# nordmtr/quantpy

Measured on AMD Instinct MI355X. Metric: state reconstructions/sec (3-qubit MLE), higher is better.
Workload: dtype f64

## Files before the change

quantpy_amd/csrc/qt_small.h:

```cpp
#pragma once
#include <hip/hip_runtime.h>
#include <stdint.h>

#include <type_traits>

#include "qt_linesearch.h"

namespace qt {

#ifdef QT_PHASE_TIMING
__device__ long long* g_qt_prof = nullptr;
#define QT_PROF_ROW \
  ((size_t)(blockIdx.x + threadIdx.y * gridDim.x) * (blockDim.x >> 6) + (threadIdx.x >> 6))
#define QT_STAMP(slot)                                                                                   \
  do {                                                                                                   \
    if (g_qt_prof && (threadIdx.x & 63) == 0)                                                            \
      g_qt_prof[QT_PROF_ROW * 32 + (slot)] = (long long)__builtin_readcyclecounter();                    \
  } while (0)
#define QT_STAMP_VAL(slot, val)                                                                          \
  do {                                                                                                   \
    if (g_qt_prof && (threadIdx.x & 63) == 0)                                                            \
      g_qt_prof[QT_PROF_ROW * 32 + (slot)] = (val);                                                      \
  } while (0)
#else
// ... 220 lines not shown
struct EstOut {
  double* rho;
  const double* centre;
  double* dist;
};

template <int NQ>
struct Small {
  static constexpr int d = 1 << NQ;
  static constexpr int D = d * d;
  static constexpr int G = D;
  static constexpr int TPW = 64 / G;
  static constexpr int WPB = 4;
  static constexpr int NT = 64 * WPB;
  static constexpr int TPB = TPW * WPB;
  static constexpr int T = d * (d - 1) / 2;
  static constexpr int LD = d == 8 ? 9 : d;
  static constexpr int MAT = 2 * LD * d;
  static constexpr int oA = 0;
  static constexpr int oB = oA + MAT;
  static constexpr int oVec = oB + MAT;
  static constexpr int oLam = oVec + D + 2;
  static constexpr int oM = oLam + 2 * ((d + 1) / 2);
  __host__ __device__ static bool v_on_rbuf(int M) { return ((M + 1) & ~1) >= MAT; }
  __host__ __device__ static int v_offset(int M, int R1) {
    const int Mp = (M + 1) & ~1;
    return v_on_rbuf(M) ? oM : oM + (R1 > 0 ? 3 : 2) * Mp;
  }
  __host__ __device__ static int trial_doubles(int M, int R1 = 0) {
    const int Mp = (M + 1) & ~1;
    return oM + (R1 > 0 ? 3 : 2) * Mp + (v_on_rbuf(M) ? 0 : MAT);
  }
  __host__ __device__ static int ipow_h(int b, int e) {
    int r = 1;
    for (int t = 0; t < e; ++t) r *= b;
    return r;
  }
  __host__ __device__ static int fwd_ints(int R1) {
    int t = 0;
    for (int q = 1; q <= NQ; ++q) t += ipow_h(R1, q) << (2 * (NQ - q));
    return t;
  }
  __host__ __device__ static int bwd_ints(int R1) {
    int t = 0;
    for (int q = 1; q <= NQ; ++q) t += ipow_h(R1, q - 1) << (2 * (NQ - q + 1));
    return t;
  }
  __host__ __device__ static int table_ints(int M, int R1) { return (fwd_ints(R1) + bwd_ints(R1) + M + 1) & ~1; }
  __host__ __device__ static int table_doubles(int M, int R1) {
    return R1 > 0 ? (table_ints(M, R1) / 2 + ((M + 1) & ~1) + 8 * R1) : 0;
  }
  __host__ __device__ static size_t lds_bytes(int M, int R1 = 0, int extra = 0) {
    return ((size_t)table_doubles(M, R1) + (size_t)TPB * (trial_doubles(M, R1) + extra)) * sizeof(double);
  }

  struct Ctx {
    int l, i, j, e;
    double* sm;
    const int *tfwd, *tbwd, *trmap;
    const double* twrow;
    const double *ttab, *ptab;
    int M, Mp;
    PovmView pv;
    int xm, zm, ny;
    int pi, pj, pkind;
    int src_re, src_im;
    __device__ __forceinline__ cd* A() const { return reinterpret_cast<cd*>(sm + oA); }
    __device__ __forceinline__ cd* Bm() const { return reinterpret_cast<cd*>(sm + oB); }
    __device__ __forceinline__ cd* V() const { return reinterpret_cast<cd*>(sm + v_offset(M, pv.pr.enabled ? pv.pr.R1 : 0)); }
    __device__ __forceinline__ double* vec() const { return sm + oVec; }
    __device__ __forceinline__ double* lam() const { return sm + oLam; }
    __device__ __forceinline__ double* rbuf() const { return sm + oM; }
    __device__ __forceinline__ double* freq() const { return sm + oM + Mp; }
    __device__ __forceinline__ double* bufB() const { return sm + oM + 2 * Mp; }
    __device__ __forceinline__ const double* tabT() const { return ttab; }
    __device__ __forceinline__ const double* tabP() const { return ptab; }
    __device__ __forceinline__ bool prod() const { return pv.pr.enabled != 0; }
    __device__ __forceinline__ double* extra() const { return sm + trial_doubles(M, pv.pr.enabled ? pv.pr.R1 : 0); }
    static constexpr bool kGeneric = true;
    static constexpr bool kHelper = false;
    __device__ __forceinline__ static constexpr int verdict_load() { return 0; }
    __device__ __forceinline__ static constexpr bool abandoned(int) { return false; }
    __device__ __forceinline__ int R1() const { return pv.pr.R1; }
    __device__ __forceinline__ bool uniform() const { return pv.pr.uniform != 0; }
    __device__ __forceinline__ bool pairedT() const { return pv.pr.pairedT != 0; }
    __device__ __forceinline__ bool pairedP() const { return pv.pr.pairedP != 0; }
    __device__ __forceinline__ double wuni() const { return pv.pr.wuni; }
    __device__ __forceinline__ double jtol2() const { return pv.jtol2; }
    __device__ __forceinline__ double cT(int k) const { return pv.pr.cT[k]; }
    __device__ __forceinline__ double cP(int k) const { return pv.pr.cP[k]; }
  };
  struct CtxS {
    int l, i, j, e;
    double* sm;
    const int* tfwd;
    const double *ttab, *ptab;
    int M, Mp;
    SpecArgs a;
    int xm, zm, ny;
    int pi, pj, pkind;
    int src_re, src_im;
    int bslot;
    double kT[12], kP[12];
    __device__ __forceinline__ cd* A() const { return reinterpret_cast<cd*>(sm + oA); }
    __device__ __forceinline__ cd* Bm() const { return reinterpret_cast<cd*>(sm + oB); }
    __device__ __forceinline__ cd* V() const { return reinterpret_cast<cd*>(sm + v_offset(M, 6)); }
    __device__ __forceinline__ double* vec() const { return sm + oVec; }
    __device__ __forceinline__ double* lam() const { return sm + oLam; }
    __device__ __forceinline__ double* rbuf() const { return sm + oM; }
    __device__ __forceinline__ double* freq() const { return sm + oM + Mp; }
    __device__ __forceinline__ double* bufB() const { return sm + oM + 2 * Mp; }
    __device__ __forceinline__ const double* tabT() const { return ttab; }
    __device__ __forceinline__ const double* tabP() const { return ptab; }
    __device__ __forceinline__ double* extra() const { return sm + trial_doubles(M, 6); }
    static constexpr bool kGeneric = false;
    static constexpr bool kHelper = false;
    __device__ __forceinline__ static constexpr int verdict_load() { return 0; }
    __device__ __forceinline__ static constexpr bool abandoned(int) { return false; }
    __device__ __forceinline__ static constexpr bool prod() { return true; }
    __device__ __forceinline__ static constexpr int R1() { return 6; }
    __device__ __forceinline__ static constexpr bool uniform() { return true; }
    __device__ __forceinline__ static constexpr bool pairedT() { return true; }
    __device__ __forceinline__ static constexpr bool pairedP() { return true; }
    __device__ __forceinline__ double wuni() const { return a.wuni; }
    __device__ __forceinline__ double jtol2() const { return a.jtol2; }
    __device__ __forceinline__ double cT(int k) const { return kT[k]; }
    __device__ __forceinline__ double cP(int k) const { return kP[k]; }
  };
  __device__ __forceinline__ static double pin_vgpr(double x) {
    asm volatile("" : "+v"(x));
    return x;
  }
  template <bool GENERIC, class = void>
  struct CtxOf {
    using type = Ctx;
  };
  template <class X>
  struct CtxOf<false, X> {
    using type = CtxS;
  };
  __host__ __device__ static int image_last_ints(int M) { return (M + 3) & ~3; }
  __host__ __device__ static int image_chunks(int M) { return image_last_ints(M) / 4 + 2 * 24 / 2; }

  __device__ __forceinline__ static int trial_index(int B, bool* live) {
    const int wave = threadIdx.x >> 6, tib = (threadIdx.x & 63) / G;
    const int b = (blockIdx.x * WPB + wave) * TPW + tib;
    *live = b < B;
    return b;
  }

  __device__ static void make_ctx(Ctx& c, double* smem_block, const PovmView& pv) {
    const int lane = threadIdx.x & 63, wave = threadIdx.x >> 6;
    c.l = lane % G;
    const int slot = wave * TPW + lane / G;
    c.i = c.l / d;
    c.j = c.l % d;
    c.e = c.i * LD + c.j;
    c.M = pv.M;
    c.Mp = (pv.M + 1) & ~1;
    c.pv = pv;
    const int r1 = pv.pr.enabled ? pv.pr.R1 : 0;
    int* tabs = reinterpret_cast<int*>(smem_block);
    c.tfwd = tabs;
    c.tbwd = tabs + fwd_ints(r1);
    c.trmap = c.tbwd + bwd_ints(r1);
    double* wrow = smem_block + table_ints(pv.M, r1) / 2;
    double* t1 = wrow + ((pv.M + 1) & ~1);
    c.twrow = wrow;
    c.ttab = t1;
    c.ptab = t1 + 4 * r1;
    if (r1 > 0) {
      const int nf = fwd_ints(r1), nb = bwd_ints(r1);
      for (int e = threadIdx.x; e < 4 * r1; e += NT) {
        t1[e] = pv.pr.T[e];
        t1[4 * r1 + e] = pv.pr.P1T[e];
      }
      if (pv.pr.pairedT) {
        for (int e = threadIdx.x; e < pv.M; e += NT) tabs[e] = pv.pr.last[e];
      } else {
        for (int e = threadIdx.x; e < nf; e += NT) tabs[e] = pv.pr.fwd[e];
      }
      if (!(pv.pr.pairedT && pv.pr.pairedP))
        for (int e = threadIdx.x; e < nb; e += NT) tabs[nf + e] = pv.pr.bwd[e];
      for (int e = threadIdx.x; e < pv.M; e += NT) {
        tabs[nf + nb + e] = pv.pr.rmap[e];
        wrow[e] = pv.pr.wrowR[e];
      }
      __syncthreads();
    }
    c.sm = smem_block + table_doubles(pv.M, r1) + slot * (trial_doubles(pv.M, r1) + pv.extra);
    int xm = 0, zm = 0, ny = 0;
#pragma unroll
    for (int b = 0; b < NQ; ++b) {
      const int dig = (c.l >> (2 * b)) & 3;
      if (dig == 1 || dig == 2) xm |= 1 << b;
      if (dig == 2 || dig == 3) zm |= 1 << b;
      if (dig == 2) ++ny;
    }
    c.xm = xm;
    c.zm = zm;
    c.ny = ny & 3;
    if (c.l < d) {
      c.pi = c.pj = c.l;
      c.pkind = 0;
    } else {
      int t = c.l - d;
      c.pkind = 1;
      if (t >= T) {
        t -= T;
        c.pkind = 2;
      }
      int ii = 1;
      while ((ii * (ii + 1)) / 2 <= t) ++ii;
      c.pi = ii;
      c.pj = t - (ii * (ii - 1)) / 2;
    }
    c.src_re = c.src_im = D;
    if (c.i == c.j) c.src_re = c.i;
    else if (c.i > c.j) {
      const int tt = (c.i * (c.i - 1)) / 2 + c.j;
      c.src_re = d + tt;
      c.src_im = d + T + tt;
    }
    if (c.l == 0) c.sm[oVec + D] = 0.0;
  }

  __device__ __forceinline__ static int pauli_index(int x, int z) {
    int k = 0;
#pragma unroll
    for (int b = 0; b < NQ; ++b) {
      const int xb = (x >> b) & 1, zb = (z >> b) & 1;
      const int dig = xb ? (zb ? 2 : 1) : (zb ? 3 : 0);
      k |= dig << (2 * b);
    }
    return k;
  }
  __device__ __forceinline__ static double re_phase(int ny, cd s) {
    return ny == 0 ? s.re : ny == 1 ? s.im : ny == 2 ? -s.re : -s.im;
  }
  __device__ __forceinline__ static cd phase_times(int ny, double v) {
    return ny == 0 ? cd{v, 0.0} : ny == 1 ? cd{0.0, -v} : ny == 2 ? cd{-v, 0.0} : cd{0.0, v};
  }

// ... 143 lines not shown
        }
      }
      wave_sync();
#pragma unroll
      for (int q = 0; q < 4; ++q) {
        const int m = c.l + q * G, mc = m < c.M ? m : c.M - 1;
        fq[mc] = raw[c.prod() ? c.trmap[mc] : mc] * inv;
      }
    } else {
      for (int m = c.l; m < c.M; m += G) {
        const double v = (double)counts[m];
        raw[m] = v;
        part += v;
      }
      total = gsum<G>(part);
      inv = 1.0 / total;
      wave_sync();
      if (c.prod()) {
        for (int m = c.l; m < c.M; m += G) fq[m] = raw[c.trmap[m]] * inv;
      } else {
        for (int m = c.l; m < c.M; m += G) fq[m] = raw[m] * inv;
      }
    }
    if (c.pv.Ns && !(pf && pf->seg)) {
      const int K = c.pv.K;
      for (int s = c.l; s < c.pv.S; s += G) {
        double t = 0.0;
        for (int k = 0; k < K; ++k) t += raw[s * K + k];
        const double ns = (pf && s == c.l) ? pf->ns[0] : c.pv.Ns[s];
        bad |= !shots_match(t, total, ns, c.pv.ns_tot);
      }
    }
    const unsigned long long votes = __builtin_amdgcn_ballot_w64(bad);
    const int lane = threadIdx.x & 63;
    const unsigned long long mine = (G == 64) ? ~0ull : (((1ull << (G & 63)) - 1ull) << (lane / G * G));
    wave_sync();
    return (votes & mine) == 0ull;
  }

  __device__ __forceinline__ static void prefetch_counts(Prefetch& pf, const int64_t* counts, const SpecArgs& a) {
    const int l = (threadIdx.x & 63) % G, M = a.M, nch = image_chunks(M), t = threadIdx.x;
    const uint4* img = reinterpret_cast<const uint4*>(a.image);
    const int* rinv = reinterpret_cast<const int*>(img + nch);
    pf.img = img[t < nch ? t : nch - 1];
    pf.ok = pf.seg = true;
#pragma unroll
    for (int q = 0; q < 4; ++q) {
      const int m = l + q * G, mc = m < M ? m : M - 1;
      pf.v[q] = counts[mc];
      pf.ri[q] = rinv[mc];
      pf.ns[q] = a.Ns[mc >> NQ];
    }
  }
  template <bool VCOEF = false>
  __device__ static void make_ctx(CtxS& c, double* smem_block, const SpecArgs& a, const Prefetch& pf) {
    const int lane = threadIdx.x & 63, wave = threadIdx.x >> 6;
    c.l = lane % G;
    const int slot = wave * TPW + lane / G;
    c.i = c.l / d;
    c.j = c.l % d;
    c.e = c.i * LD + c.j;
    c.M = a.M;
    c.Mp = (a.M + 1) & ~1;
    c.a = a;
    if ((int)threadIdx.x < image_chunks(a.M)) reinterpret_cast<uint4*>(smem_block)[threadIdx.x] = pf.img;
    c.tfwd = reinterpret_cast<const int*>(smem_block);
    c.ttab = smem_block + image_last_ints(a.M) / 2;
    c.ptab = c.ttab + 24;
    c.sm = smem_block + table_doubles(a.M, 6) + slot * (trial_doubles(a.M, 6) + a.extra);
    if (c.l == 0) c.sm[oVec + D] = 0.0;
    __syncthreads();
    int xm = 0, zm = 0, ny = 0;
#pragma unroll
    for (int b = 0; b < NQ; ++b) {
      const int dig = (c.l >> (2 * b)) & 3;
      xm |= (dig == 1 || dig == 2) << b;
      zm |= (dig >= 2) << b;
      ny += dig == 2;
    }
    c.xm = xm;
    c.zm = zm;
    c.ny = ny & 3;
    param_owner(c.l, c.pi, c.pj, c.pkind);
    const int tt = (c.i * (c.i - 1)) / 2 + c.j;
    c.src_re = c.i == c.j ? c.i : c.i > c.j ? d + tt : D;
    c.src_im = c.i > c.j ? d + T + tt : D;
    const int sx = (c.i & 1) | ((c.i & 2) << 1) | ((c.i & 4) << 2), sz = (c.j & 1) | ((c.j & 2) << 1) | ((c.j & 4) << 2);
    c.bslot = sx ^ (3 * sz);
#pragma unroll
    for (int k = 0; k < 12; ++k) {
      c.kT[k] = VCOEF ? pin_vgpr(a.cT[k]) : a.cT[k];
      c.kP[k] = VCOEF ? pin_vgpr(a.cP[k]) : a.cP[k];
    }
  }
  template <int KK>
  __device__ __forceinline__ static double gsum_above(double v) {
    if (KK < 2) v += dpp_f64<0xB1>(v);
    if (KK < 4) v += dpp_f64<0x4E>(v);
    if (G >= 8 && KK < 8) v += dpp_f64<0x141>(v);
    if (G >= 16 && KK < 16) v += dpp_f64<0x140>(v);
    if (G == 64) {
      v += dpp_f64<0x142, 0xA>(v);
      v += dpp_f64<0x143, 0xC>(v);
      v = readlane_f64(v, 63);
    }
    return v;
  }
  __device__ static bool load_freq(const CtxS& c, const Prefetch& pf) {
    double dv[4], st[4];
    bool valid[4];
#pragma unroll
    for (int q = 0; q < 4; ++q) {
      valid[q] = c.l + q * G < c.M;
      dv[q] = valid[q] ? (double)pf.v[q] : 0.0;
      st[q] = segsum_c<d>(dv[q]);
    }
    const double total = gsum_above<d>((st[0] + st[1]) + (st[2] + st[3]));
    const double inv = 1.0 / total;
    bool bad = false;
#pragma unroll
    for (int q = 0; q < 4; ++q) bad |= valid[q] & !shots_match(st[q], total, pf.ns[q], c.a.ns_tot);
    double* fq = c.freq();
// ... 327 lines not shown
        const double piv = readlane_f64(b.re, k * d + k);
        const cd bip = Vs[i * LD + k], bpj = Vs[k * LD + j];
        double inv = __builtin_amdgcn_rcp(piv);
        inv = fma(inv, fma(-piv, inv, 1.0), inv);
        inv = fma(inv, fma(-piv, inv, 1.0), inv);
        const cd t{bpj.re * inv, bpj.im * inv};
        const cd e = cmul(bip, t);
        cd nb{b.re - e.re, b.im - e.im};
        if (j == k) nb = cd{-bip.re * inv, -bip.im * inv};
        if (i == k) nb = (j == k) ? cd{inv, 0.0} : t;
        b = nb;
        if (k + 1 < d) Vs[c.e] = b;
      }
      const double mag = fabs(akk);
      const bool pos = akk > 0.0;
      if (!pos) {
        if (neg == 0) kneg = k;
        ++neg;
      }
      if (!(mag > 1e-13)) neg = neg > 0 ? 99 : neg;
      const double safe = mag > 1e-300 ? mag : 1e-300;
      if (k + 1 < d) {
        const double inv = recip_nr(safe);
        const double sinv = pos ? -inv : inv;
        const cd ajs{ajk.re * sinv, ajk.im * sinv};
        const bool upd = i > k && j > k;
        const double nre = fma(aik.re, ajs.re, fma(aik.im, ajs.im, a.re));
        const double nim = fma(aik.im, ajs.re, fma(-aik.re, ajs.im, a.im));
        a.re = upd ? nre : a.re;
        a.im = upd ? nim : a.im;
        A[c.e] = a;
        wave_sync();
      }
    }
    {
      const double dj = A[j * LD + j].re;
      const double mj = fabs(dj);
      const double rs = fast_rsqrt(mj > 1e-300 ? mj : 1e-300);
      if (i >= j) lmine = (i == j) ? cd{dj * rs, 0.0} : cd{a.re * rs, a.im * rs};
    }
    ok = neg == 0;
    if (neg_out) *neg_out = neg;
    if (kneg_out) *kneg_out = kneg;
    if (SPEC && spec_inv) *spec_inv = b;
    L[c.e] = lmine;
    wave_sync();
    const cd e = L[c.pi * LD + c.pj];
    const double x = c.pkind == 2 ? e.im : e.re;
    wave_sync();
    return x;
  }

  struct HelperLink {
    enum : int { kUnset = 0, kSpec = 1 };
    enum : int { kPending = 0, kGo = 1, kAbort = 2, kClaimed = 3, kRevoked = 4 };
    enum : int { kNothing = 0, kLifted = 1, kRefused = 2 };
    static constexpr int kHelperPolls = 1 << 15, kWaitPolls = 1 << 14, kClaimedPolls = 1 << 16;
    double* base;
    int pending;
    __device__ __forceinline__ static constexpr int doubles() { return 2 * MAT + D + 3; }
    __device__ __forceinline__ cd* image(int k) const { return reinterpret_cast<cd*>(base + k * MAT); }
    __device__ __forceinline__ cd* result() const { return image(1); }
    __device__ __forceinline__ double* x() const { return base + 2 * MAT; }
    __device__ __forceinline__ int* task() const { return reinterpret_cast<int*>(base + 2 * MAT + D); }
    __device__ __forceinline__ int* verdict() const { return task() + 1; }
    __device__ __forceinline__ int* lifted() const { return task() + 2; }
    __device__ __forceinline__ int* done() const { return task() + 3; }
    __device__ __forceinline__ int* gone() const { return task() + 4; }
    __device__ __forceinline__ int* ok() const { return task() + 5; }
    __device__ __forceinline__ static void publish(int* w, int v) {
      wave_sync();
      if ((threadIdx.x & 63) == 0) __hip_atomic_store(w, v, __ATOMIC_RELEASE, __HIP_MEMORY_SCOPE_WORKGROUP);
    }
    __device__ __forceinline__ static int peek(const int* w) {
      return __builtin_amdgcn_readfirstlane(__hip_atomic_load(w, __ATOMIC_RELAXED, __HIP_MEMORY_SCOPE_WORKGROUP));
    }
    __device__ __forceinline__ static bool claim(int* w, int from, int to) {
      int won = 0;
      if ((threadIdx.x & 63) == 0) {
        int expect = from;
        won = __hip_atomic_compare_exchange_strong(w, &expect, to, __ATOMIC_ACQ_REL, __ATOMIC_RELAXED,
                                                   __HIP_MEMORY_SCOPE_WORKGROUP);
      }
      return __builtin_amdgcn_readfirstlane(won) != 0;
    }
    template <int SLEEP>
    __device__ __forceinline__ static int poll(const int* w, int idle, int polls) {
      int v = idle;
#pragma unroll 1
      for (int n = 0; n < polls; ++n) {
        v = peek(w);
        if (v != idle) break;
        __builtin_amdgcn_s_sleep(SLEEP);
      }
      return v;
    }
    __device__ __forceinline__ void reset() {
      pending = 0;
      if ((threadIdx.x & 63) == 0) {
        *task() = kUnset;
        *verdict() = kPending;
        *lifted() = kNothing;
        *done() = 0;
        *gone() = 0;
      }
    }
    __device__ __forceinline__ void speculate(int e, cd lin) const {
      image(0)[e] = lin;
      publish(task(), kSpec);
    }
    __device__ __forceinline__ void decide(bool go) const { publish(verdict(), go ? kGo : kAbort); }
    __device__ __forceinline__ int await_lift(int e, cd& proj) {
      int v = poll<1>(lifted(), kNothing, kWaitPolls);
      if (v == kNothing) {
        if (claim(verdict(), kGo, kRevoked)) return kNothing;
        v = poll<1>(lifted(), kNothing, kClaimedPolls);
        if (v == kNothing) return kNothing;
      }
      __builtin_amdgcn_fence(__ATOMIC_ACQUIRE, "workgroup");
      if (v == kLifted) {
        proj = result()[e];
        pending = 1;
      }
      return v;
    }
    __device__ __forceinline__ bool collect(int l, double& xl, int& okl) const {
      if (poll<1>(done(), 0, kClaimedPolls) == 0) return false;
      __builtin_amdgcn_fence(__ATOMIC_ACQUIRE, "workgroup");
      xl = x()[l];
      okl = *ok();
      return true;
    }
    __device__ __forceinline__ void await_gone() const {
      poll<1>(gone(), 0, kClaimedPolls);
      __builtin_amdgcn_fence(__ATOMIC_ACQUIRE, "workgroup");
    }
  };
  struct CtxH {
    int l, i, j, e, pi, pj, pkind;
    cd *image, *second, *factor;
    const int* verdict;
    __device__ __forceinline__ cd* A() const { return image; }
    __device__ __forceinline__ cd* Bm() const { return factor; }
    __device__ __forceinline__ cd* V() const { return second; }
    __device__ __forceinline__ int verdict_load() const {
      return __hip_atomic_load(verdict, __ATOMIC_RELAXED, __HIP_MEMORY_SCOPE_WORKGROUP);
    }
    __device__ __forceinline__ static bool abandoned(int v) {
      v = __builtin_amdgcn_readfirstlane(v);
      return v != HelperLink::kPending && v != HelperLink::kGo;
    }
  };
  struct LateX {
    bool got;
    double x;
    int ok;
  };
  template <class Base>
  struct WithHelper : Base {
    HelperLink* link;
    LateX* late;
    static constexpr bool kHelper = true;
  };
  __device__ __forceinline__ static void param_owner(int l, int& pi, int& pj, int& pkind) {
    const bool diag = l < d, imag = l >= d + T;
    const int t = l - d - (imag ? T : 0);
    int ii = 1;
#pragma unroll
    for (int k = 2; k < d; ++k) ii += t >= (k * (k - 1)) / 2;
    pkind = diag ? 0 : imag ? 2 : 1;
    pi = diag ? l : ii;
    pj = diag ? l : t - (ii * (ii - 1)) / 2;
  }
  __device__ static void helper_wave(const HelperLink& k, cd* L) {
    helper_work(k, L);
    HelperLink::publish(k.gone(), 1);
  }
  __device__ static void helper_work(const HelperLink& k, cd* L) {
    static_assert(G == 64, "one trial per wavefront");
    if (HelperLink::template poll<2>(k.task(), HelperLink::kUnset, HelperLink::kHelperPolls) != HelperLink::kSpec) return;
    __builtin_amdgcn_fence(__ATOMIC_ACQUIRE, "workgroup");
    QT_STAMP(0);
    CtxH c;
    c.l = threadIdx.x & 63;
    c.i = c.l / d;
    c.j = c.l % d;
    c.e = c.i * LD + c.j;
    param_owner(c.l, c.pi, c.pj, c.pkind);
    c.image = k.image(0);
    c.second = k.image(1);
    c.factor = L;
    c.verdict = k.verdict();
    cd proj{0.0, 0.0};
    const bool lifted =
        __builtin_amdgcn_readfirstlane((int)lift_single_negative(c, c.image[c.e], d - 1, 1e-15, proj, nullptr)) != 0;
    QT_STAMP(6);
    if (HelperLink::template poll<1>(k.verdict(), HelperLink::kPending, HelperLink::kHelperPolls) != HelperLink::kGo) return;
    QT_STAMP(7);
    if (!HelperLink::claim(k.verdict(), HelperLink::kGo, HelperLink::kClaimed)) return;
    if (!lifted) {
      HelperLink::publish(k.lifted(), HelperLink::kRefused);
      return;
    }
    k.result()[c.e] = proj;
    HelperLink::publish(k.lifted(), HelperLink::kLifted);
    int ok2;
    const double x2 = cholesky_param(c, proj, ok2);
    k.x()[c.l] = x2;
    if (c.l == 0) *k.ok() = ok2;
    HelperLink::publish(k.done(), 1);
    QT_STAMP(8);
  }

  template <class C>
  __device__ static bool lift_single_negative(const C& c, cd r, int kneg, double eps, cd& out,
                                              const cd* inverse = nullptr) {
    static_assert(G == 64, "one trial per wavefront: the flags below are wave-uniform");
    cd* Ai = c.A();
    cd* Vi = c.V();
    const int i = c.i, j = c.j;
    if (i == j) r.im = 0.0;
    cd b = r;
    if (inverse) b = *inverse;
#pragma unroll 1
    for (int s = inverse ? d : 0; s < d; ++s) {
      const int p = s < kneg ? s : (s < d - 1 ? s + 1 : kneg);
      Ai[c.e] = b;
      const double piv = readlane_f64(b.re, p * d + p);
      wave_sync();
      const cd bip = Ai[i * LD + p], bpj = Ai[p * LD + j];
      wave_sync();
      double inv = __builtin_amdgcn_rcp(piv);
      inv = fma(inv, fma(-piv, inv, 1.0), inv);
      inv = fma(inv, fma(-piv, inv, 1.0), inv);
      const cd t{bpj.re * inv, bpj.im * inv};
      const cd e = cmul(bip, t);
      cd nb{b.re - e.re, b.im - e.im};
      if (j == p) nb = cd{-bip.re * inv, -bip.im * inv};
      if (i == p) nb = (j == p) ? cd{inv, 0.0} : t;
      b = nb;
    }
    QT_STAMP(4);
    b = cscale(b, fast_rsqrt(gsum<G>(b.re * b.re + b.im * b.im)));
    bool certified = false, done = false;
#pragma unroll 1
    for (int k = 1; k <= 7 && !done; ++k) {
      Ai[c.e] = b;
      wave_sync();
      [[maybe_unused]] const int verdict = c.verdict_load();
      cd n{0.0, 0.0}, n2{0.0, 0.0};
#pragma unroll
      for (int q = 0; q < d; q += 2) {
        const cd u = Ai[i * LD + q], v = Ai[j * LD + q];
        n.re = fma(u.re, v.re, fma(u.im, v.im, n.re));
        n.im = fma(u.im, v.re, fma(-u.re, v.im, n.im));
        if (q + 1 < d) {
          const cd u2 = Ai[i * LD + q + 1], v2 = Ai[j * LD + q + 1];
          n2.re = fma(u2.re, v2.re, fma(u2.im, v2.im, n2.re));
          n2.im = fma(u2.im, v2.re, fma(-u2.re, v2.im, n2.im));
        }
      }
      n = cadd(n, n2);
      wave_sync();
      if (c.abandoned(verdict)) return false;
// ... 661 lines not shown
    else if (gn != gn || fk != fk || xn != xn) status = 4;
  }
  double tr;
  const cd m = S::build_llh(c, xk, tr);
  S::emit(c, rho, b, mine, cd{m.re / tr, m.im / tr});
  if (mine) {
    if (c.l == 0) {
      if (nit_out) nit_out[b] = kiter;
      if (nfev_out) nfev_out[b] = nfev;
      if (fun_out) fun_out[b] = fk;
      if (status_out) status_out[b] = status;
    }
  }
}

#ifndef QT_BFGS_WAVES
#define QT_BFGS_WAVES 2
#endif
template <int NQ, bool GENERIC>
__global__ void __launch_bounds__(256) __attribute__((amdgpu_waves_per_eu(QT_BFGS_WAVES))) k_mle_bfgs(typename MleArgs<GENERIC>::type pv, const int64_t* __restrict__ counts, int B, int max_iter,
                                                  double gtol, EstOut rho, int32_t* __restrict__ nit_out,
                                                  int32_t* __restrict__ nfev_out, double* __restrict__ fun_out,
                                                  int32_t* __restrict__ status_out, const double* __restrict__ ws_x,
                                                  const double* __restrict__ ws_g, const double* __restrict__ ws_f,
                                                  const int32_t* __restrict__ ws_active, double* __restrict__ pairs) {
  using S = Small<NQ>;
  constexpr int D = S::D;
  bool live;
  const int b = S::trial_index(B, &live);
  const bool mine = live && ws_active[b] != 0;
  if (!__syncthreads_or(mine)) return;
  extern __shared__ __attribute__((aligned(16))) double smem[];
  typename S::template CtxOf<GENERIC>::type c;
  const int bb = live ? b : B - 1;
  if constexpr (GENERIC) {
    S::make_ctx(c, smem, pv);
    S::load_freq(c, counts + (size_t)bb * pv.M);
  } else {
    typename S::Prefetch pf;
    S::prefetch_counts(pf, counts + (size_t)bb * pv.M, pv);
    S::make_ctx(c, smem, pv, pf);
    S::load_freq(c, pf);
  }
  const double xk = mine ? ws_x[(size_t)b * D + c.l] : (c.l < S::d ? 1.0 : 0.0);
  const double gk = mine ? ws_g[(size_t)b * D + c.l] : 0.0;
  const double fk = mine ? ws_f[b] : 0.0;
  if constexpr (NQ == 3)
    bfgs_iterate_2l<NQ>(c, mine, xk, gk, fk, b, max_iter, gtol, rho, nit_out, nfev_out, fun_out, status_out, pairs);
  else
    bfgs_iterate<NQ>(c, mine, xk, gk, fk, b, max_iter, gtol, rho, nit_out, nfev_out, fun_out, status_out);
}

constexpr int kFusedLdsPairs = 24;

template <int NQ, bool GENERIC, bool HW = false>
__device__ __forceinline__ void mle_fused_body(const typename MleArgs<GENERIC>::type& pv, const int64_t* __restrict__ counts, int B, int init,
                                               int max_iter, double gtol, EstOut rho,
                                               int32_t* __restrict__ nit_out, int32_t* __restrict__ nfev_out,
                                               double* __restrict__ fun_out, int32_t* __restrict__ status_out,
                                               double* __restrict__ pairs) {
  using S = Small<NQ>;
  constexpr int D = S::D, G = S::G, d = S::d;
  extern __shared__ __attribute__((aligned(16))) double smem[];
  using Ctx = typename S::template CtxOf<GENERIC>::type;
  std::conditional_t<HW, typename S::template WithHelper<Ctx>, Ctx> c;
  [[maybe_unused]] typename S::HelperLink link;
  [[maybe_unused]] typename S::LateX late{false, 0.0, 0};
  if constexpr (HW) {
    static_assert(NQ == 3, "one trial per wavefront");
    static_assert(S::HelperLink::doubles() <= kFusedLdsPairs * 2 * D, "the hand-off lives in the LDS pair store");
    int r1 = 6;
    if constexpr (GENERIC) r1 = pv.pr.R1;
    const int per_trial = S::trial_doubles(pv.M, r1);
    double* sm = smem + S::table_doubles(pv.M, r1) + (threadIdx.x >> 6) * (per_trial + pv.extra);
    link.base = sm + per_trial + LineSearch::SLOTS + 2 * max_iter;
    if (__builtin_amdgcn_readfirstlane((int)threadIdx.y) != 0) {
      __syncthreads();
      S::helper_wave(link, reinterpret_cast<cd*>(sm + S::oB));
      return;
    }
    link.reset();
    c.link = &link;
    c.late = &late;
  }
  bool live;
  const int b = S::trial_index(B, &live);
  const int bb = live ? b : B - 1;
  typename S::Prefetch pf;
  S::prefetch_counts(pf, counts + (size_t)bb * pv.M, pv);
  bool shots_ok;
  if constexpr (GENERIC) {
    S::make_ctx(c, smem, pv);
    QT_STAMP(0);
    shots_ok = S::load_freq(c, counts + (size_t)bb * pv.M, &pf);
  } else {
    S::template make_ctx<true>(c, smem, pv, pf);
    QT_STAMP(0);
    shots_ok = S::load_freq(c, pf);
  }
  QT_STAMP(1);
  int ok;
  double xk;
  typename S::StartPoint sp;
  [[maybe_unused]] cd lin;
  if (init == 0) {
    double bl;
    lin = S::lin_invert(c, bl);
    QT_STAMP(2);
    if constexpr (HW) link.speculate(c.e, lin);
    sp.rho = S::template make_feasible<!HW>(c, lin, &xk, &ok, &sp.lscale);
  } else {
    sp.rho = cd{c.i == c.j ? 1.0 / d : 0.0, 0.0};
    sp.lscale = 1.0;
    xk = S::cholesky_param(c, sp.rho, ok);
  }
  QT_STAMP(8);
  double fk, gk;
  cd rho_l;
  [[maybe_unused]] typename S::DeferredValue dv;
  bool evaluate = true;
  if constexpr (HW) {
    if (__builtin_amdgcn_readfirstlane(link.pending)) {
      if constexpr (GENERIC) S::template nll_grad<false, decltype(c), true>(c, 0.0, fk, gk, &rho_l, true, &sp);
      else S::template nll_grad<true, decltype(c), true>(c, 0.0, fk, gk, &rho_l, true, &sp, &dv);
      xk = late.x;
      ok = late.ok;
      const bool got = __builtin_amdgcn_readfirstlane((int)late.got) != 0;
      if (!got) xk = S::cholesky_param(c, sp.rho, ok);
      ok = __builtin_amdgcn_readfirstlane(ok);
      evaluate = !got || !ok;
      if (!ok) {
        sp.rho = S::psd_project(c, lin, 1e-15);
        xk = S::cholesky_param(c, sp.rho, ok);
      }
    }
  }
  if (evaluate) {
    if constexpr (GENERIC) S::nll_grad(c, xk, fk, gk, &rho_l, true, &sp);
    else S::template nll_grad<true>(c, xk, fk, gk, &rho_l, true, &sp, &dv);
  }
  const double gnorm = gmax<G>(fabs(gk));
  QT_STAMP(9);
  const bool iterate = live && shots_ok && ok && (gnorm > gtol) && (0 < max_iter);
  if constexpr (!GENERIC) fk = S::value_if_needed(c, dv, iterate || fun_out != nullptr);
  S::emit(c, rho, b, live && !iterate, rho_l);
  if (!iterate) {
    int status = 0;
    if (!shots_ok) status = 5;
    else if (!ok) status = 1;
    else {
      const bool xnan = group_any<G>(xk != xk);
      if (0 >= max_iter) status = 3;
      else if (gnorm != gnorm || fk != fk || xnan) status = 4;
    }
    if (live) {
      if (c.l == 0) {
        if (nit_out) nit_out[b] = 0;
        if (nfev_out) nfev_out[b] = ok ? 1 : 0;
        if (fun_out) fun_out[b] = fk;
        if (status_out) status_out[b] = status;
      }
    }
  }
  QT_STAMP(10);
  if (!__any(iterate)) return;
  if (!iterate) {
    xk = (c.l < d) ? 1.0 : 0.0;
    gk = 0.0;
    fk = 0.0;
  }
  if constexpr (HW) link.await_gone();
  if constexpr (NQ == 3)
    bfgs_iterate_2l<NQ, kFusedLdsPairs>(c, iterate, xk, gk, fk, b, max_iter, gtol, rho, nit_out, nfev_out, fun_out,
                                              status_out, pairs);
  else
    bfgs_iterate<NQ>(c, iterate, xk, gk, fk, b, max_iter, gtol, rho, nit_out, nfev_out, fun_out, status_out);
}

template <int NQ, bool GENERIC>
__global__ void __launch_bounds__(256) k_mle_fused(typename MleArgs<GENERIC>::type pv, const int64_t* __restrict__ counts, int B, int max_iter,
                                                   double gtol, EstOut rho, int32_t* __restrict__ nit_out,
                                                   int32_t* __restrict__ nfev_out, double* __restrict__ fun_out,
                                                   int32_t* __restrict__ status_out, double* __restrict__ pairs) {
  mle_fused_body<NQ, GENERIC>(pv, counts, B, 0, max_iter, gtol, rho, nit_out, nfev_out, fun_out, status_out, pairs);
}
template <int NQ, bool GENERIC>
__global__ void __launch_bounds__(256) k_mle_fused_mixed(typename MleArgs<GENERIC>::type pv, const int64_t* __restrict__ counts, int B,
                                                         int max_iter, double gtol, EstOut rho,
                                                         int32_t* __restrict__ nit_out, int32_t* __restrict__ nfev_out,
                                                         double* __restrict__ fun_out, int32_t* __restrict__ status_out,
                                                         double* __restrict__ pairs) {
  mle_fused_body<NQ, GENERIC>(pv, counts, B, 1, max_iter, gtol, rho, nit_out, nfev_out, fun_out, status_out, pairs);
}

template <int NQ, bool GENERIC>
__global__ void __launch_bounds__(512) k_mle_fused_hw(typename MleArgs<GENERIC>::type pv, const int64_t* __restrict__ counts, int B, int max_iter,
                                                      double gtol, EstOut rho, int32_t* __restrict__ nit_out,
                                                      int32_t* __restrict__ nfev_out, double* __restrict__ fun_out,
                                                      int32_t* __restrict__ status_out, double* __restrict__ pairs) {
  mle_fused_body<NQ, GENERIC, true>(pv, counts, B, 0, max_iter, gtol, rho, nit_out, nfev_out, fun_out, status_out, pairs);
}

template <int NQ>
__global__ void __launch_bounds__(256) k_mhmc_state(PovmView pv, const int64_t* __restrict__ counts, int C,
                                                    const double* __restrict__ x_init, const double* __restrict__ deltas,
                                                    const double* __restrict__ uniforms, int T_steps, double step,
                                                    double* __restrict__ chain, int32_t* __restrict__ accepted) {
  using S = Small<NQ>;
  constexpr int D = S::D, G = S::G;
  extern __shared__ __attribute__((aligned(16))) double smem[];
  typename S::Ctx c;
  S::make_ctx(c, smem, pv);
  bool live;
  const int b = S::trial_index(C, &live);
  const int bb = live ? b : C - 1;
  S::load_freq(c, counts + (size_t)bb * pv.M);
  double x = x_init[(size_t)bb * D + c.l];
  double f, unused;
  S::nll_grad(c, x, f, unused, nullptr, false);
  const double* dl = deltas + (size_t)bb * T_steps * D + c.l;
  const double* un = uniforms + (size_t)bb * T_steps;
  for (int t = 0; t < T_steps; ++t) {
    const double xp = fma(step, dl[(size_t)t * D], x);
    const double nrm = sqrt(gsum<G>(xp * xp));
    const double xn = xp / nrm;
    double fn;
// ... 16 lines not shown
```

quantpy_amd/csrc/qtomo.hip:

```cpp
#include <hip/hip_runtime.h>
#include <hipcub/hipcub.hpp>
#include <stdarg.h>
#include <stdint.h>
#include <stdio.h>
#include <stdlib.h>
#include <string.h>

#include <algorithm>
#include <chrono>
#include <cmath>
#include <string>
#include <type_traits>
#include <vector>

#include "../../include/qtomo.h"
#include "qt_large.h"
#include "qt_lp.h"
#include "qt_lp_large.h"
#include "qt_ops.h"
#include "qt_polytope.h"
#include "qt_process.h"
#include "qt_process64.h"
#include "qt_process_wave16.h"
#include "qt_sampler.h"
// ... 566 lines not shown
            off(status, 1), off(x, D), off(g, D), off(f, 1), off(act, 1), M, D};
  }
};

template <int NQ, bool GENERIC>
auto mle_split_kernels() {
  if constexpr (NQ <= 3) return std::make_pair(qt::k_mle_start<NQ, GENERIC>, qt::k_mle_bfgs<NQ, GENERIC>);
  else return std::make_pair(qt::k_mle_large_start<NQ>, qt::k_mle_large_bfgs<NQ>);
}
template <bool GENERIC>
auto mle_povm_arg(const qt_handle_t* h, const Plan& p) {
  if constexpr (GENERIC) return p.pv;
  else return h->spec_args(p.pv.extra);
}

int mle_batch_impl(qt_handle_t* h, const int64_t* counts, int B, int init, int max_iter, double tol, const double* centre,
                   double* rho, double* dist, int32_t* nit, int32_t* nfev, double* fun, int32_t* status, int flags) {
  QT_ENTER(h);
  Call c(h, flags);
  if (int r = need_povm(h)) return r;
  if (B < 0 || (B > 0 && (!counts || (!rho && !dist) || (dist && !centre)))) return fail(QT_ERR_ARG, "bad mle_batch arguments");
  if (init != QT_INIT_LIN && init != QT_INIT_MIXED) return fail(QT_ERR_ARG, "init must be QT_INIT_LIN or QT_INIT_MIXED");
  if (max_iter < 0) return fail(QT_ERR_ARG, "max_iter < 0");
  if (B == 0) return 0;
  const int64_t* dc;
  const double* dcen;
  double *drho, *dfun, *ddist;
  int32_t *dnit, *dnfev, *dst;
  const size_t nel = (size_t)B * h->D;
  if (int r = c.in(counts, (size_t)B * h->M, &dc)) return r;
  if (int r = c.in(centre, (size_t)h->D * 2, &dcen)) return r;
  if (int r = c.out(rho, nel * 2, &drho)) return r;
  if (int r = c.out(nit, (size_t)B, &dnit)) return r;
  if (int r = c.out(nfev, (size_t)B, &dnfev)) return r;
  if (int r = c.out(fun, (size_t)B, &dfun)) return r;
  if (int r = c.out(status, (size_t)B, &dst)) return r;
  if (int r = c.out(dist, (size_t)B, &ddist)) return r;
  const qt::EstOut eo{drho, dcen, ddist};
  if (h->nq >= 4) {
    if (int r = prepare_large(h, init == QT_INIT_LIN)) return r;
    if (max_iter > 4096) return fail(QT_ERR_UNSUPPORTED, "max_iter > 4096 is not supported for n_qubits >= 4");
  }
  if (h->nq == 3 && max_iter > 2000)
    return fail(QT_ERR_UNSUPPORTED, "max_iter > 2000 is not supported for n_qubits = 3 (LDS holds the two-loop scalars)");
  const int mi = max_iter > 0 ? max_iter : 1;
  h->last_mle_spec = h->spec_eligible();
  h->last_mle_helper = false;
  return by_nq(h, [&](auto nq) -> int {
    constexpr int NQ = decltype(nq)::value;
    if constexpr (NQ <= 3) {
      constexpr int TPW = qt::Small<NQ>::TPW;
      if ((B + TPW - 1) / TPW <= h->fused_max_waves && !(NQ == 3 && max_iter > 256)) {
        int extra = 0;
        if (NQ == 3) {
          extra = qt::LineSearch::SLOTS + 2 * mi + qt::kFusedLdsPairs * 2 * h->D;
          const int over = mi > qt::kFusedLdsPairs ? mi : 1;
          HIPCHK(h->hess.ensure((size_t)B * over * 2 * h->D * sizeof(double)));
        }
        Plan p = povm_plan<NQ>(h, B, extra);
        auto fused = [&](auto generic) {
          constexpr bool GEN = decltype(generic)::value;
          if constexpr (NQ == 3) {
            if (h->mle_helper_wave && init == QT_INIT_LIN && p.pv.pr.enabled) {
              h->last_mle_helper = true;
              p.block = dim3(qt::Small<NQ>::NT, 2);
              return launch(h, qt::k_mle_fused_hw<NQ, GEN>, p, mle_povm_arg<GEN>(h, p), dc, B, max_iter, tol, eo, dnit, dnfev,
                            dfun, dst, h->hess.as<double>());
            }
          }
          return launch(h, init == QT_INIT_LIN ? qt::k_mle_fused<NQ, GEN> : qt::k_mle_fused_mixed<NQ, GEN>, p,
                        mle_povm_arg<GEN>(h, p), dc, B, max_iter, tol, eo, dnit, dnfev, dfun, dst, h->hess.as<double>());
        };
        if (int r = h->last_mle_spec ? fused(std::false_type()) : fused(std::true_type())) return r;
        return c.done(status, B);
      }
    }
    HIPCHK(h->ws_x.ensure(nel * sizeof(double)));
    HIPCHK(h->ws_g.ensure(nel * sizeof(double)));
    HIPCHK(h->ws_f.ensure((size_t)B * sizeof(double)));
    HIPCHK(h->ws_act.ensure((size_t)B * sizeof(int32_t)));
    int chunk = B;
    if (NQ >= 3) {
      const size_t per_trial = (size_t)mi * 2 * h->D * sizeof(double);
      chunk = (int)(((size_t)4 << 30) / per_trial);
      if (chunk < 1) chunk = 1;
      if (chunk > B) chunk = B;
      HIPCHK(h->hess.ensure((size_t)chunk * per_trial));
    }
    const MleArrays all{dc, eo, dnit, dnfev, dfun, dst, h->ws_x.as<double>(), h->ws_g.as<double>(), h->ws_f.as<double>(),
                        h->ws_act.as<int32_t>(), h->M, h->D};
    auto split = [&](auto generic) -> int {
      constexpr bool GEN = decltype(generic)::value || NQ >= 4;
      const auto [k_start, k_bfgs] = mle_split_kernels<NQ, GEN>();
      const Plan ps = povm_plan<NQ>(h, B);
      if (int r = launch(h, k_start, ps, mle_povm_arg<GEN>(h, ps), dc, B, init, max_iter, tol, eo, dnit, dnfev, dfun, dst, all.x,
                         all.g, all.f, all.act))
        return r;
      const int extra = NQ >= 4 ? max_iter : (NQ == 3 ? qt::LineSearch::SLOTS + 2 * mi : 0);
      for (int b0 = 0; b0 < B; b0 += chunk) {
        const int nb = B - b0 < chunk ? B - b0 : chunk;
        const MleArrays a = all.at(b0);
        const Plan p = povm_plan<NQ>(h, nb, extra);
        if (int r = launch(h, k_bfgs, p, mle_povm_arg<GEN>(h, p), a.counts, nb, max_iter, tol, a.eo, a.nit, a.nfev, a.fun,
                           a.status, a.x, a.g, a.f, a.act, h->hess.as<double>()))
          return r;
      }
      return c.done(status, B);
    };
    return h->last_mle_spec ? split(std::false_type()) : split(std::true_type());
  });
}

int project(qt_handle_t* h, const double* in, int B, int mode, int n_iter, double tol, double* out, int32_t* iters,
            int32_t* status, const double* centre = nullptr, double* dist = nullptr) {
  if (h->D == 64) {
    if (mode != 1) HIPCHK(h->proc_ws.ensure((size_t)B * qt::Proc64::kWsComplex * 2 * sizeof(double)));
    return launch(h, qt::k_cptp_project64, dim3(B), dim3(qt::Proc64::NT), qt::Proc64::kLdsBytes, in, B, mode, n_iter, tol, out,
                  iters, status, h->proc_ws.as<double>());
// ... 1543 lines not shown
```

Before: 98.73 million.

## Make helper wave a full twin that races the lift with its own LDS slot

The helper wave (threadIdx.y=1) becomes a twin trial context with its own LDS scratch region. It runs the linear inversion itself and then attempts the single-negative-eigenvalue lift directly, instead of waiting for a speculated image from the main wave. When the twin's lift is claimed, the main wave does the Cholesky sweep and exits, and the twin carries on with BFGS. The LDS pair store shrinks from 24 to 16 pairs to fit the extra twin slot, and the twin runs at raised priority. This is meant to remove the hand-off latency from the critical path, at the cost of duplicated work, more LDS per block and a smaller in-LDS BFGS history.

```diff
diff --git a/quantpy_amd/csrc/qt_small.h b/quantpy_amd/csrc/qt_small.h
--- a/quantpy_amd/csrc/qt_small.h
+++ b/quantpy_amd/csrc/qt_small.h
@@ -296,6 +296,12 @@
   }
   __host__ __device__ static size_t lds_bytes(int M, int R1 = 0, int extra = 0) {
     return ((size_t)table_doubles(M, R1) + (size_t)TPB * (trial_doubles(M, R1) + extra)) * sizeof(double);
+  }
+  __host__ __device__ static int twin_offset(int M, int R1, int extra) {
+    return table_doubles(M, R1) + TPB * (trial_doubles(M, R1) + extra);
+  }
+  __host__ __device__ static size_t lds_bytes_twin(int M, int R1, int extra) {
+    return lds_bytes(M, R1, extra) + (size_t)TPB * trial_doubles(M, R1) * sizeof(double);
   }
 
   struct Ctx {
@@ -393,7 +399,8 @@
     return b;
   }
 
-  __device__ static void make_ctx(Ctx& c, double* smem_block, const PovmView& pv) {
+  template <bool TWIN = false>
+  __device__ static void make_ctx(Ctx& c, double* smem_block, const PovmView& pv, [[maybe_unused]] int twin = 0) {
     const int lane = threadIdx.x & 63, wave = threadIdx.x >> 6;
     c.l = lane % G;
     const int slot = wave * TPW + lane / G;
@@ -415,24 +422,27 @@
     c.ptab = t1 + 4 * r1;
     if (r1 > 0) {
       const int nf = fwd_ints(r1), nb = bwd_ints(r1);
-      for (int e = threadIdx.x; e < 4 * r1; e += NT) {
-        t1[e] = pv.pr.T[e];
-        t1[4 * r1 + e] = pv.pr.P1T[e];
-      }
-      if (pv.pr.pairedT) {
-        for (int e = threadIdx.x; e < pv.M; e += NT) tabs[e] = pv.pr.last[e];
-      } else {
-        for (int e = threadIdx.x; e < nf; e += NT) tabs[e] = pv.pr.fwd[e];
-      }
-      if (!(pv.pr.pairedT && pv.pr.pairedP))
-        for (int e = threadIdx.x; e < nb; e += NT) tabs[nf + e] = pv.pr.bwd[e];
-      for (int e = threadIdx.x; e < pv.M; e += NT) {
-        tabs[nf + nb + e] = pv.pr.rmap[e];
-        wrow[e] = pv.pr.wrowR[e];
+      if (!(TWIN && twin)) {
+        for (int e = threadIdx.x; e < 4 * r1; e += NT) {
+          t1[e] = pv.pr.T[e];
+          t1[4 * r1 + e] = pv.pr.P1T[e];
+        }
+        if (pv.pr.pairedT) {
+          for (int e = threadIdx.x; e < pv.M; e += NT) tabs[e] = pv.pr.last[e];
+        } else {
+          for (int e = threadIdx.x; e < nf; e += NT) tabs[e] = pv.pr.fwd[e];
+        }
+        if (!(pv.pr.pairedT && pv.pr.pairedP))
+          for (int e = threadIdx.x; e < nb; e += NT) tabs[nf + e] = pv.pr.bwd[e];
+        for (int e = threadIdx.x; e < pv.M; e += NT) {
+          tabs[nf + nb + e] = pv.pr.rmap[e];
+          wrow[e] = pv.pr.wrowR[e];
+        }
       }
       __syncthreads();
     }
     c.sm = smem_block + table_doubles(pv.M, r1) + slot * (trial_doubles(pv.M, r1) + pv.extra);
+    if (TWIN && twin) c.sm = smem_block + twin_offset(pv.M, r1, pv.extra) + slot * trial_doubles(pv.M, r1);
     int xm = 0, zm = 0, ny = 0;
 #pragma unroll
     for (int b = 0; b < NQ; ++b) {
@@ -682,8 +692,9 @@
       pf.ns[q] = a.Ns[mc >> NQ];
     }
   }
-  template <bool VCOEF = false>
-  __device__ static void make_ctx(CtxS& c, double* smem_block, const SpecArgs& a, const Prefetch& pf) {
+  template <bool VCOEF = false, bool TWIN = false>
+  __device__ static void make_ctx(CtxS& c, double* smem_block, const SpecArgs& a, const Prefetch& pf,
+                                  [[maybe_unused]] int twin = 0) {
     const int lane = threadIdx.x & 63, wave = threadIdx.x >> 6;
     c.l = lane % G;
     const int slot = wave * TPW + lane / G;
@@ -693,11 +704,12 @@
     c.M = a.M;
     c.Mp = (a.M + 1) & ~1;
     c.a = a;
-    if ((int)threadIdx.x < image_chunks(a.M)) reinterpret_cast<uint4*>(smem_block)[threadIdx.x] = pf.img;
+    if (!(TWIN && twin) && (int)threadIdx.x < image_chunks(a.M)) reinterpret_cast<uint4*>(smem_block)[threadIdx.x] = pf.img;
     c.tfwd = reinterpret_cast<const int*>(smem_block);
     c.ttab = smem_block + image_last_ints(a.M) / 2;
     c.ptab = c.ttab + 24;
     c.sm = smem_block + table_doubles(a.M, 6) + slot * (trial_doubles(a.M, 6) + a.extra);
+    if (TWIN && twin) c.sm = smem_block + twin_offset(a.M, 6, a.extra) + slot * trial_doubles(a.M, 6);
     if (c.l == 0) c.sm[oVec + D] = 0.0;
     __syncthreads();
     int xm = 0, zm = 0, ny = 0;
@@ -1131,22 +1143,19 @@
   }
 
   struct HelperLink {
-    enum : int { kUnset = 0, kSpec = 1 };
     enum : int { kPending = 0, kGo = 1, kAbort = 2, kClaimed = 3, kRevoked = 4 };
     enum : int { kNothing = 0, kLifted = 1, kRefused = 2 };
     static constexpr int kHelperPolls = 1 << 15, kWaitPolls = 1 << 14, kClaimedPolls = 1 << 16;
     double* base;
     int pending;
-    __device__ __forceinline__ static constexpr int doubles() { return 2 * MAT + D + 3; }
-    __device__ __forceinline__ cd* image(int k) const { return reinterpret_cast<cd*>(base + k * MAT); }
-    __device__ __forceinline__ cd* result() const { return image(1); }
-    __device__ __forceinline__ double* x() const { return base + 2 * MAT; }
-    __device__ __forceinline__ int* task() const { return reinterpret_cast<int*>(base + 2 * MAT + D); }
-    __device__ __forceinline__ int* verdict() const { return task() + 1; }
-    __device__ __forceinline__ int* lifted() const { return task() + 2; }
-    __device__ __forceinline__ int* done() const { return task() + 3; }
-    __device__ __forceinline__ int* gone() const { return task() + 4; }
-    __device__ __forceinline__ int* ok() const { return task() + 5; }
+    __device__ __forceinline__ static constexpr int doubles() { return MAT + D + 3; }
+    __device__ __forceinline__ cd* result() const { return reinterpret_cast<cd*>(base); }
+    __device__ __forceinline__ double* x() const { return base + MAT; }
+    __device__ __forceinline__ int* verdict() const { return reinterpret_cast<int*>(base + MAT + D); }
+    __device__ __forceinline__ int* lifted() const { return verdict() + 1; }
+    __device__ __forceinline__ int* done() const { return verdict() + 2; }
+    __device__ __forceinline__ int* gone() const { return verdict() + 3; }
+    __device__ __forceinline__ int* ok() const { return verdict() + 4; }
     __device__ __forceinline__ static void publish(int* w, int v) {
       wave_sync();
       if ((threadIdx.x & 63) == 0) __hip_atomic_store(w, v, __ATOMIC_RELEASE, __HIP_MEMORY_SCOPE_WORKGROUP);
@@ -1177,16 +1186,11 @@
     __device__ __forceinline__ void reset() {
       pending = 0;
       if ((threadIdx.x & 63) == 0) {
-        *task() = kUnset;
         *verdict() = kPending;
         *lifted() = kNothing;
         *done() = 0;
         *gone() = 0;
       }
-    }
-    __device__ __forceinline__ void speculate(int e, cd lin) const {
-      image(0)[e] = lin;
-      publish(task(), kSpec);
     }
     __device__ __forceinline__ void decide(bool go) const { publish(verdict(), go ? kGo : kAbort); }
     __device__ __forceinline__ int await_lift(int e, cd& proj) {
@@ -1239,6 +1243,8 @@
   struct WithHelper : Base {
     HelperLink* link;
     LateX* late;
+    double* xtra;
+    __device__ __forceinline__ double* extra() const { return xtra; }
     static constexpr bool kHelper = true;
   };
   __device__ __forceinline__ static void param_owner(int l, int& pi, int& pj, int& pkind) {
@@ -1251,44 +1257,49 @@
     pi = diag ? l : ii;
     pj = diag ? l : t - (ii * (ii - 1)) / 2;
   }
-  __device__ static void helper_wave(const HelperLink& k, cd* L) {
-    helper_work(k, L);
-    HelperLink::publish(k.gone(), 1);
-  }
-  __device__ static void helper_work(const HelperLink& k, cd* L) {
+  template <class C>
+  __device__ static bool twin_lift(const C& t, const HelperLink& k, cd lin, cd& proj) {
     static_assert(G == 64, "one trial per wavefront");
-    if (HelperLink::template poll<2>(k.task(), HelperLink::kUnset, HelperLink::kHelperPolls) != HelperLink::kSpec) return;
-    __builtin_amdgcn_fence(__ATOMIC_ACQUIRE, "workgroup");
-    QT_STAMP(0);
-    CtxH c;
-    c.l = threadIdx.x & 63;
-    c.i = c.l / d;
-    c.j = c.l % d;
-    c.e = c.i * LD + c.j;
-    param_owner(c.l, c.pi, c.pj, c.pkind);
-    c.image = k.image(0);
-    c.second = k.image(1);
-    c.factor = L;
-    c.verdict = k.verdict();
-    cd proj{0.0, 0.0};
-    const bool lifted =
-        __builtin_amdgcn_readfirstlane((int)lift_single_negative(c, c.image[c.e], d - 1, 1e-15, proj, nullptr)) != 0;
+    CtxH c = side_ctx(t, k, t.Bm());
+    proj = cd{0.0, 0.0};
+    const bool lifted = __builtin_amdgcn_readfirstlane((int)lift_single_negative(c, lin, d - 1, 1e-15, proj, nullptr)) != 0;
     QT_STAMP(6);
-    if (HelperLink::template poll<1>(k.verdict(), HelperLink::kPending, HelperLink::kHelperPolls) != HelperLink::kGo) return;
+    if (HelperLink::template poll<1>(k.verdict(), HelperLink::kPending, HelperLink::kHelperPolls) != HelperLink::kGo) return false;
     QT_STAMP(7);
-    if (!HelperLink::claim(k.verdict(), HelperLink::kGo, HelperLink::kClaimed)) return;
+    if (!HelperLink::claim(k.verdict(), HelperLink::kGo, HelperLink::kClaimed)) return false;
     if (!lifted) {
       HelperLink::publish(k.lifted(), HelperLink::kRefused);
-      return;
+      return false;
     }
     k.result()[c.e] = proj;
     HelperLink::publish(k.lifted(), HelperLink::kLifted);
+    return true;
+  }
+  template <class C>
+  __device__ static void sweep_for(const C& t, const HelperLink& k, cd proj, cd* L) {
+    CtxH c = side_ctx(t, k, L);
     int ok2;
     const double x2 = cholesky_param(c, proj, ok2);
     k.x()[c.l] = x2;
     if (c.l == 0) *k.ok() = ok2;
     HelperLink::publish(k.done(), 1);
-    QT_STAMP(8);
+    QT_STAMP(7);
+  }
+  template <class C>
+  __device__ __forceinline__ static CtxH side_ctx(const C& t, const HelperLink& k, cd* L) {
+    CtxH c;
+    c.l = t.l;
+    c.i = t.i;
+    c.j = t.j;
+    c.e = t.e;
+    c.pi = t.pi;
+    c.pj = t.pj;
+    c.pkind = t.pkind;
+    c.image = t.A();
+    c.second = t.V();
+    c.factor = L;
+    c.verdict = k.verdict();
+    return c;
   }
 
   template <class C>
@@ -2056,6 +2067,7 @@
 }
 
 constexpr int kFusedLdsPairs = 24;
+constexpr int kFusedHwLdsPairs = 16;
 
 template <int NQ, bool GENERIC, bool HW = false>
 __device__ __forceinline__ void mle_fused_body(const typename MleArgs<GENERIC>::type& pv, const int64_t* __restrict__ counts, int B, int init,
@@ -2070,21 +2082,22 @@
   std::conditional_t<HW, typename S::template WithHelper<Ctx>, Ctx> c;
   [[maybe_unused]] typename S::HelperLink link;
   [[maybe_unused]] typename S::LateX late{false, 0.0, 0};
+  [[maybe_unused]] int twin = 0;
+  [[maybe_unused]] double* trial_sm = nullptr;
   if constexpr (HW) {
     static_assert(NQ == 3, "one trial per wavefront");
-    static_assert(S::HelperLink::doubles() <= kFusedLdsPairs * 2 * D, "the hand-off lives in the LDS pair store");
+    static_assert(S::HelperLink::doubles() <= kFusedHwLdsPairs * 2 * D, "the hand-off lives in the LDS pair store");
     int r1 = 6;
     if constexpr (GENERIC) r1 = pv.pr.R1;
     const int per_trial = S::trial_doubles(pv.M, r1);
-    double* sm = smem + S::table_doubles(pv.M, r1) + (threadIdx.x >> 6) * (per_trial + pv.extra);
-    link.base = sm + per_trial + LineSearch::SLOTS + 2 * max_iter;
-    if (__builtin_amdgcn_readfirstlane((int)threadIdx.y) != 0) {
-      __syncthreads();
-      S::helper_wave(link, reinterpret_cast<cd*>(sm + S::oB));
-      return;
-    }
-    link.reset();
+    trial_sm = smem + S::table_doubles(pv.M, r1) + (threadIdx.x >> 6) * (per_trial + pv.extra);
+    link.base = trial_sm + per_trial + LineSearch::SLOTS + 2 * max_iter;
+    twin = __builtin_amdgcn_readfirstlane((int)threadIdx.y);
+    link.pending = 0;
+    if (!twin) link.reset();
+    if (twin) __builtin_amdgcn_s_setprio(1);
     c.link = &link;
+    c.xtra = trial_sm + per_trial;
     c.late = &late;
   }
   bool live;
@@ -2094,11 +2107,11 @@
   S::prefetch_counts(pf, counts + (size_t)bb * pv.M, pv);
   bool shots_ok;
   if constexpr (GENERIC) {
-    S::make_ctx(c, smem, pv);
+    S::template make_ctx<HW>(c, smem, pv, twin);
     QT_STAMP(0);
     shots_ok = S::load_freq(c, counts + (size_t)bb * pv.M, &pf);
   } else {
-    S::template make_ctx<true>(c, smem, pv, pf);
+    S::template make_ctx<true, HW>(c, smem, pv, pf, twin);
     QT_STAMP(0);
     shots_ok = S::load_freq(c, pf);
   }
@@ -2111,8 +2124,29 @@
     double bl;
     lin = S::lin_invert(c, bl);
     QT_STAMP(2);
-    if constexpr (HW) link.speculate(c.e, lin);
-    sp.rho = S::template make_feasible<!HW>(c, lin, &xk, &ok, &sp.lscale);
+    bool feasible = false;
+    if constexpr (HW) {
+      if (twin) {
+        if (!S::twin_lift(c, link, lin, sp.rho)) {
+          S::HelperLink::publish(link.gone(), 1);
+          return;
+        }
+        sp.lscale = 1.0;
+        link.pending = 1;
+        feasible = true;
+      }
+    }
+    if (!feasible) sp.rho = S::template make_feasible<!HW>(c, lin, &xk, &ok, &sp.lscale);
+    if constexpr (HW) {
+      if (!twin && __builtin_amdgcn_readfirstlane(link.pending)) {
+        int r1 = 6;
+        if constexpr (GENERIC) r1 = pv.pr.R1;
+        double* twin_sm = smem + S::twin_offset(pv.M, r1, pv.extra) + (threadIdx.x >> 6) * S::trial_doubles(pv.M, r1);
+        S::sweep_for(c, link, sp.rho, reinterpret_cast<cd*>(twin_sm + S::oB));
+        S::HelperLink::publish(link.gone(), 1);
+        return;
+      }
+    }
   } else {
     sp.rho = cd{c.i == c.j ? 1.0 / d : 0.0, 0.0};
     sp.lscale = 1.0;
@@ -2175,7 +2209,7 @@
   }
   if constexpr (HW) link.await_gone();
   if constexpr (NQ == 3)
-    bfgs_iterate_2l<NQ, kFusedLdsPairs>(c, iterate, xk, gk, fk, b, max_iter, gtol, rho, nit_out, nfev_out, fun_out,
+    bfgs_iterate_2l<NQ, HW ? kFusedHwLdsPairs : kFusedLdsPairs>(c, iterate, xk, gk, fk, b, max_iter, gtol, rho, nit_out, nfev_out, fun_out,
                                               status_out, pairs);
   else
     bfgs_iterate<NQ>(c, iterate, xk, gk, fk, b, max_iter, gtol, rho, nit_out, nfev_out, fun_out, status_out);
diff --git a/quantpy_amd/csrc/qtomo.hip b/quantpy_amd/csrc/qtomo.hip
--- a/quantpy_amd/csrc/qtomo.hip
+++ b/quantpy_amd/csrc/qtomo.hip
@@ -642,18 +642,26 @@
       constexpr int TPW = qt::Small<NQ>::TPW;
       if ((B + TPW - 1) / TPW <= h->fused_max_waves && !(NQ == 3 && max_iter > 256)) {
         int extra = 0;
+        bool helper = false;
+        size_t lds_hw = 0;
         if (NQ == 3) {
-          extra = qt::LineSearch::SLOTS + 2 * mi + qt::kFusedLdsPairs * 2 * h->D;
-          const int over = mi > qt::kFusedLdsPairs ? mi : 1;
+          const int state = qt::LineSearch::SLOTS + 2 * mi;
+          const int extra_hw = state + qt::kFusedHwLdsPairs * 2 * h->D;
+          lds_hw = qt::Small<3>::lds_bytes_twin(h->M, h->prod.R1, extra_hw);
+          helper = h->mle_helper_wave && init == QT_INIT_LIN && h->prod.enabled && lds_hw <= kLdsLimit;
+          const int lds_pairs = helper ? qt::kFusedHwLdsPairs : qt::kFusedLdsPairs;
+          extra = state + lds_pairs * 2 * h->D;
+          const int over = mi > lds_pairs ? mi : 1;
           HIPCHK(h->hess.ensure((size_t)B * over * 2 * h->D * sizeof(double)));
         }
         Plan p = povm_plan<NQ>(h, B, extra);
         auto fused = [&](auto generic) {
           constexpr bool GEN = decltype(generic)::value;
           if constexpr (NQ == 3) {
-            if (h->mle_helper_wave && init == QT_INIT_LIN && p.pv.pr.enabled) {
+            if (helper) {
               h->last_mle_helper = true;
               p.block = dim3(qt::Small<NQ>::NT, 2);
+              p.lds = lds_hw;
               return launch(h, qt::k_mle_fused_hw<NQ, GEN>, p, mle_povm_arg<GEN>(h, p), dc, B, max_iter, tol, eo, dnit, dnfev,
                             dfun, dst, h->hess.as<double>());
             }
```

After: 100.4 million (median of 6 runs). 1.6% higher.
